# Harvard-AI-and-Robotics-Lab/FairFedMed

Measured on AMD Instinct MI355X. Metric: images/sec per client-round, ViT-B/16 FairLoRA r=8, bs=32 224^2, higher is better.
Workload: dtype bf16; 1 GPU; configs[1]: 1-client ViT-B/16 FairLoRA rank=8 G=3, bs=32 synthetic 224x224x3, fwd+bwd+SGD per step; global_batch=32, clients=1, trainable_elems=741952, loss_finite=1, launch=replay, rccl_ranks=1

## Files before the change

fairfedmed_amd/csrc/lora.hip:

```cpp
#include "common.h"

namespace {

constexpr int LD_WAVES = 8;
constexpr int LD_LDS_BUDGET = 64 * 1024;

template <int V>
__device__ __forceinline__ void reduce_scatter64(float (&vals)[V], int lane) {
#pragma unroll
    for (int n = V, o = 32; o >= 1; n >>= 1, o >>= 1) {
        const bool up = (lane & o) != 0;
#pragma unroll
        for (int i = 0; i < n / 2; ++i) {
            const float a = vals[i], b = vals[i + n / 2];
            const float keep = up ? b : a, send = up ? a : b;
            vals[i] = keep + __shfl_xor(send, o, 64);
        }
    }
}

template <typename T, int RP>
__global__ __launch_bounds__(LD_WAVES * 64) void lora_down_kernel(
    const T* __restrict__ x, int ldx, const float* __restrict__ P, int layout_rk, const float* __restrict__ S,
    const int32_t* __restrict__ attr, int M, int K, int r, int G, int rows_per_sample, float scaling,
// ... 226 lines not shown
        d_uni[e] = rows16(d_uni[e]);
    }
    if (col == 0) {
#pragma unroll
        for (int e = 0; e < 4; ++e) {
            dsum[0 * 16 + 4 * kgp + e] = d_all[e];
            dsum[1 * 16 + 4 * kgp + e] = d_uni[e];
        }
    }
    for (int g = 0; g < G; ++g) {
#pragma unroll
        for (int e = 0; e < 4; ++e) {
            const float o = rows16(ga == g ? wv[e] : 0.f);
            if (col == 0) dsum[(2 + g) * 16 + 4 * kgp + e] = o;
        }
    }
    __builtin_amdgcn_s_waitcnt(0xc07f);
    __builtin_amdgcn_wave_barrier();
    if (lane < G * r) {
        const int g = lane / r, j = lane % r;
        ds_part[((size_t)blockIdx.x * G + g) * r + j] = w_uni * dsum[16 + j] + w_oth * dsum[j] + (w_own - w_oth) * dsum[(2 + g) * 16 + j];
    }
    for (int i = lane + 64; i < G * r; i += 64) {
        const int g = i / r, j = i % r;
        ds_part[((size_t)blockIdx.x * G + g) * r + j] = w_uni * dsum[16 + j] + w_oth * dsum[j] + (w_own - w_oth) * dsum[(2 + g) * 16 + j];
    }
}

static bool down_mfma_ok(int M, int K, int r, int dtype, int layout_rk) {
    return dtype == FFM_BF16 && layout_rk && r <= 16 && M >= 1024 && K % (32 * LDM_WAVES) == 0;
}

static int down_kq(int K, int es) {
    const int nch = K * es / 16;
    return nch >= 256 ? 4 : nch >= 96 ? 2 : 1;
}
static int down_rp(int r, int dtype) { return r <= 4 && dtype == FFM_F32 ? 4 : r <= 8 ? 8 : 16; }

template <typename T, int RP>
int launch_down(const void* x, int ldx, const float* P, int layout_rk, const float* S, const int32_t* attr, int M,
                int K, int r, int G, int rps, float scaling, float lam, float* t, float* ts, const float* t_fwd,
                float* ds_part, int rs, int j0, hipStream_t s) {
    constexpr int CE = Elem<T>::kPerChunk;
    int ktile = K;
    const int per_col = RP * (int)sizeof(T);
    if (K * per_col > LD_LDS_BUDGET) ktile = (LD_LDS_BUDGET / per_col) / (64 * CE) * (64 * CE);
    const int lds = ktile * per_col;
    const int kq = down_kq(K, (int)sizeof(T));
    const int rows = (LD_WAVES / kq) * (64 / RP);
    const int blocks = (M + rows - 1) / rows;
    hipLaunchKernelGGL((lora_down_kernel<T, RP>), dim3(blocks), dim3(LD_WAVES * 64), lds, s, (const T*)x, ldx, P,
                       layout_rk, S, attr, M, K, r, G, rps, scaling, lam, t, ts, t_fwd, ds_part, ktile, rs, j0, kq);
    FFM_CHECK_LAUNCH();
    return FFM_OK;
}

constexpr int LG_WAVES = 4;
constexpr int LG_RPW = 32;
constexpr int LG_ROWS = LG_WAVES * LG_RPW;

template <typename T, int RP>
__global__ __launch_bounds__(LG_WAVES * 64) void lora_grad_kernel(const T* __restrict__ x, int ldx,
                                                                   const float* __restrict__ v, int M, int K, int r,
                                                                   float* __restrict__ part, int rs, int j0) {
    constexpr int CE = Elem<T>::kPerChunk;
    extern __shared__ __attribute__((aligned(16))) char smem[];
    float* red = reinterpret_cast<float*>(smem);
    const int lane = threadIdx.x & 63;
    const int wave = __builtin_amdgcn_readfirstlane(threadIdx.x >> 6);
    const int k = (blockIdx.x * 64 + lane) * CE;
    const int split = blockIdx.y;
    const bool active = k < K;
    const int m0 = split * LG_ROWS + wave * LG_RPW;
    const int m1 = (m0 + LG_RPW) < M ? (m0 + LG_RPW) : M;

    float acc[CE][RP];
#pragma unroll
    for (int e = 0; e < CE; ++e)
#pragma unroll
        for (int j = 0; j < RP; ++j) acc[e][j] = 0.f;

    const T* xc = x + (active ? k : 0);
    for (int m = m0; m < m1; m += 8) {
        typename Elem<T>::chunk_t xv[8];
#pragma unroll
        for (int u = 0; u < 8; ++u) {
            const int mm = (m + u) < m1 ? (m + u) : (m1 - 1);
            xv[u] = *reinterpret_cast<const typename Elem<T>::chunk_t*>(xc + (size_t)mm * ldx);
        }
#pragma unroll
        for (int u = 0; u < 8; ++u) {
            if (m + u < m1) {
                const float* vr = v + (size_t)(m + u) * rs + j0;
                float vj[RP];
#pragma unroll
                for (int j = 0; j < RP; ++j) vj[j] = (j < r) ? vr[j] : 0.f;
#pragma unroll
                for (int e = 0; e < CE; ++e) {
                    const float xe = Elem<T>::to_f(xv[u][e]);
#pragma unroll
                    for (int j = 0; j < RP; ++j) acc[e][j] += xe * vj[j];
                }
            }
        }
    }
    if (wave >= 2) {
#pragma unroll
        for (int e = 0; e < CE; ++e)
#pragma unroll
            for (int j = 0; j < RP; ++j) red[((wave - 2) * CE * RP + e * RP + j) * 64 + lane] = acc[e][j];
    }
    __syncthreads();
    if (wave < 2) {
#pragma unroll
        for (int e = 0; e < CE; ++e)
#pragma unroll
            for (int j = 0; j < RP; ++j) acc[e][j] += red[(wave * CE * RP + e * RP + j) * 64 + lane];
    }
    __syncthreads();
    if (wave == 1) {
#pragma unroll
        for (int e = 0; e < CE; ++e)
#pragma unroll
            for (int j = 0; j < RP; ++j) red[(e * RP + j) * 64 + lane] = acc[e][j];
    }
    __syncthreads();
    if (wave == 0 && active) {
        float* dst = part + ((size_t)split * K + k) * rs + j0;
#pragma unroll
        for (int e = 0; e < CE; ++e)
#pragma unroll
            for (int j = 0; j < RP; ++j)
                if (j < r) dst[e * rs + j] = acc[e][j] + red[(e * RP + j) * 64 + lane];
    }
}

template <typename T, int RP>
int launch_grad(const void* x, int ldx, const float* v, int M, int K, int r, float* part, int rs, int j0,
                hipStream_t s) {
    constexpr int CE = Elem<T>::kPerChunk;
    dim3 grid((K + 64 * CE - 1) / (64 * CE), (M + LG_ROWS - 1) / LG_ROWS);
    const int lds = 2 * CE * RP * 64 * 4;
    if (lds > 65536) {
        hipError_t e = hipFuncSetAttribute(reinterpret_cast<const void*>(lora_grad_kernel<T, RP>),
                                           hipFuncAttributeMaxDynamicSharedMemorySize, lds);
        if (e != hipSuccess) return (int)e;
    }
    hipLaunchKernelGGL((lora_grad_kernel<T, RP>), grid, dim3(LG_WAVES * 64), lds, s, (const T*)x, ldx, v, M, K, r,
                       part, rs, j0);
    FFM_CHECK_LAUNCH();
    return FFM_OK;
}

constexpr int LGM_ROWS = 128, LGM_COLS = 128;

__device__ __forceinline__ int lgm_swz(int row) { return ((row & 3) << 2) | ((row >> 2) & 3); }

struct lgm_ln {
    const float *mean, *rstd, *gamma, *beta;
};

template <int RP, bool LN>
__global__ __launch_bounds__(64) void lora_grad_mfma_kernel(const bf16_t* __restrict__ x, int ldx,
                                                            const float* __restrict__ v, int M, int K, int r,
                                                            float* __restrict__ part, int rs, int j0, lgm_ln ln) {
    extern __shared__ __attribute__((aligned(16))) char smem[];
    const int lane = threadIdx.x;
    const int k0 = blockIdx.x * LGM_COLS, split = blockIdx.y, m0 = split * LGM_ROWS;

#ifdef FFM_LGM_NOLDS
    {
        bf16x8 sink = {};
#pragma unroll 8
        for (int piece = 0; piece < LGM_ROWS / 4; ++piece) {
            const int row = piece * 4 + (lane >> 4);
            int gm = m0 + row;
            gm = gm < M ? gm : M - 1;
            const bf16x8 t = *reinterpret_cast<const bf16x8*>(x + (size_t)gm * ldx + k0 + (lane & 15) * 8);
#pragma unroll
            for (int e = 0; e < 8; ++e) sink[e] = (bf16_t)((float)sink[e] + (float)t[e]);
        }
        if (v[0] == 123456.f) part[lane] = (float)sink[0];
        return;
    }
#endif
#pragma unroll
    for (int piece = 0; piece < LGM_ROWS / 4; ++piece) {
        const int row = piece * 4 + (lane >> 4);
        int gm = m0 + row;
        gm = gm < M ? gm : M - 1;
        const int ch = (lane & 15) ^ lgm_swz(row);
        const bf16_t* src = x + (size_t)gm * ldx + k0 + ch * 8;
        __builtin_amdgcn_global_load_lds((const __attribute__((address_space(1))) void*)src,
                                         (__attribute__((address_space(3))) void*)(smem + piece * 1024), 16, 0, 0);
    }
    const int j = lane & 15, kg = lane >> 4;
    bf16x8 ahi[4], alo[4];
    float s1 = 0.f, s2 = 0.f;
#pragma unroll
    for (int rb = 0; rb < 4; ++rb) {
        float vv[8];
#pragma unroll
        for (int t = 0; t < 8; ++t) {
            const int gm = m0 + rb * 32 + kg * 8 + t;
            vv[t] = (j < r && gm < M) ? v[(size_t)gm * rs + j0 + j] : 0.f;
            if constexpr (LN) {
                const int gc = gm < M ? gm : M - 1;
                const float rsd = ln.rstd[gc];
                s2 += vv[t];
                vv[t] *= rsd;
                s1 += ln.mean[gc] * vv[t];
            }
        }
#pragma unroll
        for (int t = 0; t < 8; ++t) {
            const bf16_t h = (bf16_t)vv[t];
            ahi[rb][t] = h;
            alo[rb][t] = (bf16_t)(vv[t] - (float)h);
        }
    }
    asm volatile("s_waitcnt vmcnt(0)" ::: "memory");
    __builtin_amdgcn_s_barrier();

    const int q = (lane & 15) >> 2, pp = lane & 3;
    f32x4 acc[LGM_COLS / 16];
#pragma unroll
    for (int cf = 0; cf < LGM_COLS / 16; ++cf) acc[cf] = (f32x4){0.f, 0.f, 0.f, 0.f};
    typedef __attribute__((ext_vector_type(2))) uint32_t u32x2;
    typedef __attribute__((ext_vector_type(4))) uint32_t u32x4;
#pragma unroll
    for (int rb = 0; rb < 4; ++rb) {
        const int R = rb * 32 + kg * 8 + q;
        const uint32_t base0 = (uint32_t)(uintptr_t)smem + 256 * R + 8 * (pp & 1);
        const uint32_t base1 = base0 + 256 * 4;
        const int s0 = lgm_swz(R), s1 = lgm_swz(R + 4);
        u32x2 lo2[LGM_COLS / 16], hi2[LGM_COLS / 16];
#pragma unroll
        for (int cf = 0; cf < LGM_COLS / 16; ++cf) {
            const int ch = cf * 2 + (pp >> 1);
            asm volatile("ds_read_b64_tr_b16 %0, %1" : "=v"(lo2[cf]) : "v"(base0 + 16 * (ch ^ s0)) : "memory");
            asm volatile("ds_read_b64_tr_b16 %0, %1" : "=v"(hi2[cf]) : "v"(base1 + 16 * (ch ^ s1)) : "memory");
        }
        asm volatile("s_waitcnt lgkmcnt(0)" ::: "memory");
#pragma unroll
        for (int cf = 0; cf < LGM_COLS / 16; ++cf) {
            asm volatile("" : "+v"(lo2[cf]), "+v"(hi2[cf]));
            const u32x4 packed = {lo2[cf][0], lo2[cf][1], hi2[cf][0], hi2[cf][1]};
            const bf16x8 b = __builtin_bit_cast(bf16x8, packed);
            acc[cf] = __builtin_amdgcn_mfma_f32_16x16x32_bf16(ahi[rb], b, acc[cf], 0, 0, 0);
            acc[cf] = __builtin_amdgcn_mfma_f32_16x16x32_bf16(alo[rb], b, acc[cf], 0, 0, 0);
        }
    }
    (void)RP;
    float c1[4] = {0.f, 0.f, 0.f, 0.f}, c2[4] = {0.f, 0.f, 0.f, 0.f};
    if constexpr (LN) {
        s1 += __shfl_xor(s1, 16, 64);
        s1 += __shfl_xor(s1, 32, 64);
        s2 += __shfl_xor(s2, 16, 64);
        s2 += __shfl_xor(s2, 32, 64);
#pragma unroll
        for (int e = 0; e < 4; ++e) {
            c1[e] = __shfl(s1, 4 * kg + e, 64);
            c2[e] = __shfl(s2, 4 * kg + e, 64);
        }
    }
#pragma unroll
    for (int cf = 0; cf < LGM_COLS / 16; ++cf) {
        const int k = k0 + cf * 16 + (lane & 15);
        float* dst = part + ((size_t)split * K + k) * rs + j0;
        float gk = 1.f, bk = 0.f;
        if constexpr (LN) { gk = ln.gamma[k]; bk = ln.beta[k]; }
#pragma unroll
        for (int e = 0; e < 4; ++e) {
            const int jj = 4 * kg + e;
            if (jj < r) dst[jj] = LN ? gk * (acc[cf][e] - c1[e]) + bk * c2[e] : acc[cf][e];
        }
    }
}

int launch_grad_mfma(const void* x, int ldx, const float* v, int M, int K, int r, float* part, int rs, int j0,
                     hipStream_t s, const lgm_ln* ln = nullptr) {
    dim3 grid(K / LGM_COLS, (M + LGM_ROWS - 1) / LGM_ROWS);
#ifdef FFM_LGM_NOLDS
#define LGM_LDS 0
#else
#define LGM_LDS (LGM_ROWS * LGM_COLS * 2)
#endif
    if (ln)
        hipLaunchKernelGGL((lora_grad_mfma_kernel<16, true>), grid, dim3(64), LGM_LDS, s, (const bf16_t*)x, ldx,
                           v, M, K, r, part, rs, j0, *ln);
    else
        hipLaunchKernelGGL((lora_grad_mfma_kernel<16, false>), grid, dim3(64), LGM_LDS, s, (const bf16_t*)x, ldx,
                           v, M, K, r, part, rs, j0, lgm_ln{});
    FFM_CHECK_LAUNCH();
    return FFM_OK;
}

__global__ __launch_bounds__(256) void reduce_partials_kernel(const float* __restrict__ part, int nsplit, int n,
                                                              float* __restrict__ out, int tK, int tr,
                                                              int accumulate) {
    const int gid = blockIdx.x * blockDim.x + threadIdx.x;
    const int i = (gid >> 2);
    const int q = gid & 3;
    float s = 0.f;
    if (i < n)
        for (int sp = q; sp < nsplit; sp += 4) s += part[(size_t)sp * n + i];
    s += __shfl_xor(s, 1, 64);
    s += __shfl_xor(s, 2, 64);
    if (i >= n || q != 0) return;
    int o = i;
    if (tK > 0) {
        const int k = i / tr, j = i % tr;
        o = j * tK + k;
    }
    out[o] = accumulate ? out[o] + s : s;
}

__global__ __launch_bounds__(1024) void reduce_partials_tall_kernel(const float* __restrict__ part, int nsplit, int n,
                                                                    float* __restrict__ out, int tK, int tr, int accumulate) {
    __shared__ float red[16][64];
    const int lane = threadIdx.x & 63, wave = threadIdx.x >> 6;
    const int i = blockIdx.x * 64 + lane;
    float s0 = 0.f, s1 = 0.f, s2 = 0.f, s3 = 0.f;
    if (i < n) {
        int sp = wave;
        for (; sp + 48 < nsplit; sp += 64) {
            s0 += part[(size_t)sp * n + i];
            s1 += part[(size_t)(sp + 16) * n + i];
            s2 += part[(size_t)(sp + 32) * n + i];
            s3 += part[(size_t)(sp + 48) * n + i];
        }
        for (; sp < nsplit; sp += 16) s0 += part[(size_t)sp * n + i];
    }
    red[wave][lane] = (s0 + s1) + (s2 + s3);
    __syncthreads();
    if (wave != 0 || i >= n) return;
    float s = 0.f;
#pragma unroll
    for (int w = 0; w < 16; ++w) s += red[w][lane];
    int o = i;
    if (tK > 0) {
        const int k = i / tr, j = i % tr;
        o = j * tK + k;
    }
    out[o] = accumulate ? out[o] + s : s;
}

__global__ __launch_bounds__(256) void reduce_multi_kernel(const ffm_reduce_desc* __restrict__ descs) {
    const ffm_reduce_desc d = descs[blockIdx.y];
    const int L = d.nsplit > 64 ? 32 : 4, sh = d.nsplit > 64 ? 5 : 2;
    if ((long long)blockIdx.x * blockDim.x >= (long long)L * d.n) return;
    const int gid = blockIdx.x * blockDim.x + threadIdx.x;
    const int i = gid >> sh, q = gid & (L - 1);
    float s = 0.f;
    if (i < d.n)
        for (int sp = q; sp < d.nsplit; sp += L) s += d.part[(size_t)sp * d.n + i];
    s += __shfl_xor(s, 1, 64);
    s += __shfl_xor(s, 2, 64);
    if (L == 32) {
        s += __shfl_xor(s, 4, 64);
        s += __shfl_xor(s, 8, 64);
        s += __shfl_xor(s, 16, 64);
    }
    if (i >= d.n || q != 0) return;
    int o = i;
    if (d.transpose_K > 0) {
        const int k = i / d.transpose_r, j = i % d.transpose_r;
        o = j * d.transpose_K + k;
    }
    d.out[o] = s;
}

}

static int down_valu_blocks(int M, int K, int r, int dtype) {
    const int rows = (LD_WAVES / down_kq(K, dtype == FFM_BF16 ? 2 : 4)) * (64 / down_rp(r, dtype));
    return (M + rows - 1) / rows;
}
extern "C" int ffm_lora_down_blocks(int M, int K, int r, int dtype) {
    if (down_mfma_ok(M, K, r, dtype, 1)) return (M + LDM_ROWS - 1) / LDM_ROWS;
    return down_valu_blocks(M, K, r, dtype);
}
extern "C" int ffm_lora_down_blocks_max(int M_max, int K, int r, int dtype) {
    const int valu = down_valu_blocks(M_max, K, r, dtype);
    const int mf = down_mfma_ok(M_max, K, r, dtype, 1) ? (M_max + LDM_ROWS - 1) / LDM_ROWS : 0;
    return mf > valu ? mf : valu;
}
extern "C" int ffm_lora_grad_splits(int M) { return (M + LG_ROWS - 1) / LG_ROWS; }

extern "C" int ffm_lora_down(const void* x, int ldx, const float* P, int layout_rk, const float* S,
                             const int32_t* attr, int M, int K, int r, int G, int rows_per_sample, float scaling,
                             float lambda_group, float* t, float* ts, const float* t_fwd, float* ds_part, int dtype,
                             void* stream) {
    if (!x || !P || !S || M <= 0 || K <= 0 || r <= 0 || r > FFM_MAX_RANK || G <= 0 || G > FFM_MAX_GROUPS ||
        rows_per_sample <= 0)
        return FFM_EINVAL;
    if ((t_fwd == nullptr) != (ds_part == nullptr)) return FFM_EINVAL;
    if (G * r > 256) return FFM_EUNSUP;
    const size_t es = dtype == FFM_BF16 ? 2 : 4;
    if (dtype != FFM_BF16 && dtype != FFM_F32) return FFM_EINVAL;
    if (((size_t)K * es) % 16 || ((size_t)ldx * es) % 16 || ((uintptr_t)x & 15)) return FFM_EINVAL;
    hipStream_t s = (hipStream_t)stream;
    if (down_mfma_ok(M, K, r, dtype, layout_rk)) {
        hipLaunchKernelGGL(lora_down_mfma_kernel, dim3((M + LDM_ROWS - 1) / LDM_ROWS), dim3(LDM_WAVES * 64), 0, s, (const bf16_t*)x,
                           ldx, P, S, attr, M, K, r, G, rows_per_sample, scaling, lambda_group, t, ts, t_fwd, ds_part);
        FFM_CHECK_LAUNCH();
        return FFM_OK;
    }
#define DOWN(RP, RR, J0) launch_down<T, RP>(x, ldx, P, layout_rk, S, attr, M, K, RR, G, rows_per_sample, scaling, \
                                            lambda_group, t, ts, t_fwd, ds_part, r, J0, s)
    return ffm_by_storage(dtype, [&](auto tag) {
        typedef typename decltype(tag)::type T;
        if (r > 16) {
            int e = DOWN(16, 16, 0);
            if (e) return e;
            return DOWN(16, r - 16, 16);
        }
        if constexpr (sizeof(T) == 4) {
            if (r <= 4) return DOWN(4, r, 0);
        }
        return r <= 8 ? DOWN(8, r, 0) : DOWN(16, r, 0);
    });
#undef DOWN
}

extern "C" int ffm_lora_grad_partial(const void* x, int ldx, const float* v, int M, int K, int r, float* part,
                                     int dtype, void* stream) {
    if (!x || !v || !part || M <= 0 || K <= 0 || r <= 0 || r > FFM_MAX_RANK) return FFM_EINVAL;
    const size_t es = dtype == FFM_BF16 ? 2 : 4;
    if (dtype != FFM_BF16 && dtype != FFM_F32) return FFM_EINVAL;
    if (((size_t)K * es) % 16 || ((size_t)ldx * es) % 16 || ((uintptr_t)x & 15)) return FFM_EINVAL;
    hipStream_t s = (hipStream_t)stream;
    if (dtype == FFM_BF16 && K % LGM_COLS == 0) {
        for (int j0 = 0; j0 < r; j0 += 16) {
            const int e = launch_grad_mfma(x, ldx, v, M, K, (r - j0) < 16 ? (r - j0) : 16, part, r, j0, s);
            if (e) return e;
        }
        return FFM_OK;
    }
#define GRAD(RP, RR, J0) launch_grad<T, RP>(x, ldx, v, M, K, RR, part, r, J0, s)
    return ffm_by_storage(dtype, [&](auto tag) {
        typedef typename decltype(tag)::type T;
        if (r > 16) {
            int e = GRAD(16, 16, 0);
            if (e) return e;
            return GRAD(16, r - 16, 16);
        }
        return r <= 4 ? GRAD(4, r, 0) : r <= 8 ? GRAD(8, r, 0) : GRAD(16, r, 0);
    });
#undef GRAD
}

extern "C" int ffm_lora_grad_partial_ln(const void* x, int ldx, const float* v, const float* mean, const float* rstd,
                                        const float* gamma, const float* beta, int M, int K, int r, float* part,
                                        int dtype, void* stream) {
    if (!x || !v || !mean || !rstd || !gamma || !beta || !part || M <= 0 || K <= 0 || r <= 0) return FFM_EINVAL;
    if (dtype != FFM_BF16 || K % LGM_COLS || r > 16) return FFM_EUNSUP;
    if (((size_t)ldx * 2) % 16 || ((uintptr_t)x & 15)) return FFM_EINVAL;
    const lgm_ln ln = {mean, rstd, gamma, beta};
    return launch_grad_mfma(x, ldx, v, M, K, r, part, r, 0, (hipStream_t)stream, &ln);
}

extern "C" int ffm_reduce_partials_multi(const ffm_reduce_desc* descs_dev, int ndesc, int max_n, void* stream) {
    if (!descs_dev || ndesc <= 0 || max_n <= 0) return FFM_EINVAL;
    hipLaunchKernelGGL(reduce_multi_kernel, dim3((4 * max_n + 255) / 256, ndesc), dim3(256), 0, (hipStream_t)stream,
                       descs_dev);
    FFM_CHECK_LAUNCH();
    return FFM_OK;
}

extern "C" int ffm_reduce_partials(const float* part, int nsplit, int n, float* out, int transpose_K,
                                   int transpose_r, int accumulate, void* stream) {
    if (!part || !out || nsplit <= 0 || n <= 0) return FFM_EINVAL;
    if (transpose_K > 0 && (transpose_r <= 0 || transpose_K * transpose_r != n)) return FFM_EINVAL;
    if (nsplit >= 512 && (long long)n * 16 < (long long)nsplit * 64)
        hipLaunchKernelGGL(reduce_partials_tall_kernel, dim3((n + 63) / 64), dim3(1024), 0, (hipStream_t)stream, part, nsplit, n,
                           out, transpose_K, transpose_r, accumulate);
    else
        hipLaunchKernelGGL(reduce_partials_kernel, dim3((4 * n + 255) / 256), dim3(256), 0, (hipStream_t)stream, part,
                           nsplit, n, out, transpose_K, transpose_r, accumulate);
    FFM_CHECK_LAUNCH();
    return FFM_OK;
}
```

fairfedmed_amd/ops.py:

```python
from __future__ import annotations

import ctypes as C
from typing import Optional

import torch

from . import _lib as L

Tensor = torch.Tensor

_REC = None


class record:
    def __init__(self, plan: list):
        self.plan = plan

    def __enter__(self):
        global _REC
        self.prev, _REC = _REC, self.plan
        return self.plan

    def __exit__(self, *a):
        global _REC
# ... 513 lines not shown
    _call("ffm_eval_counts", L.ptr(prob), L.ptr(label), L.ptr(attr), N, num_groups, L.ptr(out), L.stream_ptr())
    return out


EVAL_BOOT_WS_BUDGET = 256 << 20
EVAL_BOOT_MAX_CHUNK = 65535


def eval_boot_chunk(N: int, B: int) -> int:
    size = L.load().ffm_eval_boot_ws_bytes
    if int(size(N, 1)) <= 0:
        raise RuntimeError("ffm_eval_boot_ws_bytes failed")
    lo, hi = 1, int(max(1, min(B, EVAL_BOOT_MAX_CHUNK)))
    while lo < hi:
        mid = (lo + hi + 1) // 2
        if int(size(N, mid)) <= EVAL_BOOT_WS_BUDGET:
            lo = mid
        else:
            hi = mid - 1
    return lo


def eval_boot_counts(prob: Tensor, label: Tensor, attr: Optional[Tensor], num_groups: int, B: int, seed: int, tag: int = 0,
                     chunk: Optional[int] = None, out: Optional[Tensor] = None) -> Tensor:
    _dev(prob, label, attr)
    N = prob.shape[0]
    assert prob.dtype == torch.float32 and prob.dim() == 2 and prob.shape[1] == 2 and prob.is_contiguous()
    assert label.dtype == torch.int64 and label.is_contiguous() and label.numel() == N
    assert attr is None or (attr.dtype == torch.int64 and attr.is_contiguous() and attr.numel() == N)
    B = int(B)
    if B <= 0:
        raise ValueError(f"eval_boot_counts needs B >= 1 replicates, got {B}")
    if recording():
        raise RuntimeError("eval_boot_counts holds a temporary workspace and cannot be recorded")
    if chunk is None:
        chunk = eval_boot_chunk(N, B)
    chunk = int(chunk)
    if not 1 <= chunk <= EVAL_BOOT_MAX_CHUNK:
        raise ValueError(f"eval_boot_counts: chunk must lie in 1..{EVAL_BOOT_MAX_CHUNK}, got {chunk}")
    if out is None:
        out = torch.empty(B, num_groups + 2, EVAL_SLOTS, device=prob.device, dtype=torch.int64)
    assert out.dtype == torch.int64 and out.is_contiguous() and tuple(out.shape) == (B, num_groups + 2, EVAL_SLOTS) and out.is_cuda
    nbytes = int(L.load().ffm_eval_boot_ws_bytes(N, chunk))
    if nbytes <= 0:
        raise RuntimeError("ffm_eval_boot_ws_bytes failed")
    ws = torch.empty(nbytes + 256, device=prob.device, dtype=torch.uint8)
    off = (-ws.data_ptr()) % 256
    _call("ffm_eval_boot_counts", L.ptr(prob), L.ptr(label), L.ptr(attr), N, num_groups, B, chunk, int(seed), int(tag),
          L.ptr(out), ws.data_ptr() + off, nbytes, L.stream_ptr())
    return out


def attention_fwd(qkv: Tensor, out: Tensor, lse: Optional[Tensor], B: int, Ltok: int, heads: int,
                  causal: bool = False) -> Tensor:
    _dev(qkv, out, lse)
    assert qkv.is_contiguous() and out.is_contiguous() and qkv.dtype == out.dtype
    assert qkv.shape[1] == 3 * heads * 64 and out.shape[1] == heads * 64
    _call("ffm_attention_fwd", L.ptr(qkv), L.ptr(out), L.ptr(_f32(lse)), B, Ltok, heads, int(causal),
                                       L.dtype_code(qkv.dtype), L.stream_ptr())
    return out


def attention_bwd_lnstat_ok(Ltok: int, causal: bool, dtype: torch.dtype) -> bool:
    return L.is16(dtype) and bool(L.load().ffm_attention_bwd_lnstat_ok(Ltok, int(causal), L.dtype_code(dtype)))


def attention_bwd(qkv: Tensor, out: Tensor, dout: Tensor, lse: Tensor, delta: Tensor, dqkv: Tensor, B: int,
                  Ltok: int, heads: int, causal: bool = False, ln_stat: Optional[tuple] = None) -> Tensor:
    _dev(qkv, out, dout, lse, delta, dqkv)
    for t in (qkv, out, dout, dqkv):
        assert t.is_contiguous() and t.dtype == qkv.dtype
    if ln_stat is not None:
        wg, d, part = ln_stat
        _dev(wg, d, part)
        E3 = 3 * heads * 64
        assert _f32(wg).numel() == E3 and _f32(d).numel() == E3 and _f32(part).numel() >= 2 * heads * B * Ltok * 2
        _call("ffm_attention_bwd_lnstat", L.ptr(qkv), L.ptr(out), L.ptr(dout), L.ptr(_f32(lse)), L.ptr(_f32(delta)), L.ptr(dqkv),
              L.ptr(wg), L.ptr(d), L.ptr(part), B, Ltok, heads, int(causal), L.dtype_code(qkv.dtype), L.stream_ptr())
        return dqkv
    _call("ffm_attention_bwd", L.ptr(qkv), L.ptr(out), L.ptr(dout), L.ptr(_f32(lse)), L.ptr(_f32(delta)),
                                       L.ptr(dqkv), B, Ltok, heads, int(causal), L.dtype_code(qkv.dtype),
                                       L.stream_ptr())
    return dqkv


def lora_down_blocks(M: int, K: int, r: int, dtype: torch.dtype) -> int:
    return L.load().ffm_lora_down_blocks(M, K, r, L.dtype_code(dtype))


def lora_down_blocks_max(M_max: int, K: int, r: int, dtype: torch.dtype) -> int:
    return L.load().ffm_lora_down_blocks_max(M_max, K, r, L.dtype_code(dtype))


class ReducePlan:

    def __init__(self, entries, device):
        import ctypes as C
        arr = (L.ReduceDesc * len(entries))()
        self.keep = entries
        self.max_n = 0
        for i, (part, nsplit, n, out, tK, tr) in enumerate(entries):
            _dev(part, out)
            arr[i] = L.ReduceDesc(part.data_ptr(), out.data_ptr(), nsplit, n, tK, tr)
            self.max_n = max(self.max_n, n * (8 if nsplit > 64 else 1))
        raw = bytes(arr)
        self.table = torch.frombuffer(bytearray(raw), dtype=torch.uint8).to(device)
        self.n = len(entries)

    def run(self) -> None:
        _call("ffm_reduce_partials_multi", self.table.data_ptr(), self.n, self.max_n, L.stream_ptr())


class PackPlan:

    def __init__(self, entries, dtype, device):
        arr = (L.PackDesc * len(entries))()
        self.keep, self.max_K, self.dtype = entries, 0, dtype
        self.any_ln = False
        for i, ent in enumerate(entries):
            src, layout_rk, dst = ent[:3]
            wide = ent[3] if len(ent) > 3 else None
            ln = ent[4] if len(ent) > 4 else None
            _dev(src, dst, wide)
            K = dst.shape[1]
            r = src.shape[0] if layout_rk else src.shape[1]
            assert dst.dtype == dtype and dst.shape[0] == 16 and dst.is_contiguous() and src.is_contiguous()
            assert wide is None or (wide.dtype == dtype and tuple(wide.shape) == (K, 32) and wide.is_contiguous())
            lnp = (None, None, None)
            if ln is not None:
                assert not layout_rk and _f32(ln[0]).numel() == K and _f32(ln[1]).numel() == K and _f32(ln[2]).numel() == 32
                _dev(*ln)
                lnp = tuple(t.data_ptr() for t in ln)
                self.any_ln = True
            rows = ent[5] if len(ent) > 5 and ent[5] is not None else (None, None)
            if rows[0] is not None:
                _dev(*rows)
                assert r <= 14 and _f32(rows[0]).numel() == K and _f32(rows[1]).numel() == K
            arr[i] = L.PackDesc(src.data_ptr(), dst.data_ptr(), K, r, int(layout_rk), 0, L.ptr(wide), *lnp, L.ptr(rows[0]), L.ptr(rows[1]))
            self.max_K = max(self.max_K, K)
        self.table = torch.frombuffer(bytearray(bytes(arr)), dtype=torch.uint8).to(device)
        self.n = len(entries)

    def run(self) -> None:
        _call("ffm_lora_pack_multi", self.table.data_ptr(), self.n, self.max_K, L.dtype_code(self.dtype),
                                             L.stream_ptr())
        if self.any_ln:
            _call("ffm_lora_pack_ln", self.table.data_ptr(), self.n, L.dtype_code(self.dtype), L.stream_ptr())


def lora_grad_partial_ln(x: Tensor, v: Tensor, mean: Tensor, rstd: Tensor, gamma: Tensor, beta: Tensor, r: int,
                         part: Tensor) -> None:
    _dev(x, v, mean, rstd, gamma, beta, part)
    M, K = x.shape
    assert L.is16(x.dtype) and K % 128 == 0 and r <= 16
    _call("ffm_lora_grad_partial_ln", L.ptr(x), _ld(x), L.ptr(_f32(v)), L.ptr(_f32(mean)), L.ptr(_f32(rstd)),
          L.ptr(_f32(gamma)), L.ptr(_f32(beta)), M, K, r, L.ptr(_f32(part)), L.dtype_code(x.dtype), L.stream_ptr())


def lora_grad_splits(M: int) -> int:
    return L.load().ffm_lora_grad_splits(M)


def lora_down(x: Tensor, P: Tensor, layout_rk: bool, S: Tensor, attr: Optional[Tensor], r: int, G: int,
              rows_per_sample: int, scaling: float, lambda_group: float, t: Optional[Tensor], ts: Optional[Tensor],
              t_fwd: Optional[Tensor] = None, ds_part: Optional[Tensor] = None) -> None:
    _dev(x, P, S, attr, t, ts, t_fwd, ds_part)
    M, K = x.shape
    if attr is not None:
        assert attr.dtype == torch.int32
    _call("ffm_lora_down", L.ptr(x), _ld(x), L.ptr(_f32(P)), int(layout_rk), L.ptr(_f32(S)), L.ptr(attr), M,
                                   K, r, G, rows_per_sample, scaling, lambda_group, L.ptr(_f32(t)), L.ptr(_f32(ts)),
                                   L.ptr(_f32(t_fwd)), L.ptr(_f32(ds_part)), L.dtype_code(x.dtype), L.stream_ptr())


def lora_grad_partial(x: Tensor, v: Tensor, r: int, part: Tensor) -> None:
    _dev(x, v, part)
    M, K = x.shape
    _call("ffm_lora_grad_partial", L.ptr(x), _ld(x), L.ptr(_f32(v)), M, K, r, L.ptr(_f32(part)),
                                           L.dtype_code(x.dtype), L.stream_ptr())


def reduce_partials(part: Tensor, nsplit: int, n: int, out: Tensor, transpose_K: int = 0, transpose_r: int = 0,
                    accumulate: bool = False) -> None:
    _dev(part, out)
    _call("ffm_reduce_partials", L.ptr(_f32(part)), nsplit, n, L.ptr(out), transpose_K, transpose_r,
                                         int(accumulate), L.stream_ptr())


def head_fwd(f: Tensor, tbar: Tensor, logit_scale: Tensor, fbar: Tensor, rnorm: Tensor, logits_img: Tensor, B: int,
             Ltok: int, n_cls: int) -> None:
    _dev(f, tbar, logit_scale, fbar, rnorm, logits_img)
    D = f.shape[1]
    assert f.is_contiguous()
    _call("ffm_head_fwd", L.ptr(f), L.ptr(_f32(tbar)), L.ptr(_f32(logit_scale)), L.ptr(_f32(fbar)),
                                  L.ptr(_f32(rnorm)), L.ptr(_f32(logits_img)), B, Ltok, D, n_cls,
                                  L.dtype_code(f.dtype), L.stream_ptr())


def text_embed(prefix: Tensor, ctx: Tensor, suffix: Tensor, pos: Tensor, x: Tensor, n_cls: int, TL: int) -> None:
    _dev(prefix, ctx, suffix, pos, x)
    n_prompts, n_ctx, w = ctx.shape
    for t in (prefix, ctx, suffix, pos, x):
        assert t.dtype == torch.float32 and t.is_contiguous()
    assert prefix.shape[0] == suffix.shape[0] == n_prompts * n_cls and x.shape[0] >= n_prompts * n_cls * TL and pos.shape[0] >= TL
    _call("ffm_text_embed", L.ptr(prefix), L.ptr(ctx), L.ptr(suffix), suffix.shape[1], L.ptr(pos), L.ptr(x), n_prompts, n_cls,
          n_ctx, TL, w, L.stream_ptr())


def text_tail_fwd(x: Tensor, eot_row: Tensor, lnw: Tensor, lnb: Tensor, proj: Tensor, tf: Tensor, tn: Tensor, rnorm: Tensor,
                  stats: Tensor, tbar: Optional[Tensor], n_prompts: int, n_cls: int) -> None:
    _dev(x, eot_row, lnw, lnb, proj, tf, tn, rnorm, stats, tbar)
    assert eot_row.dtype == torch.int32 and x.dtype == torch.float32 and proj.dtype == torch.float32 and proj.is_contiguous()
    w, D = proj.shape
    assert x.shape[1] == w and tf.shape == tn.shape == (n_prompts * n_cls, D) and tf.is_contiguous() and tn.is_contiguous()
    _call("ffm_text_tail_fwd", L.ptr(x), L.ptr(eot_row), L.ptr(lnw), L.ptr(lnb), L.ptr(proj), L.ptr(tf), L.ptr(tn), L.ptr(rnorm),
          L.ptr(stats), L.ptr(tbar), n_prompts, n_cls, w, D, L.stream_ptr())


def text_tail_bwd(x: Tensor, eot_row: Tensor, lnw: Tensor, proj: Tensor, tn: Tensor, rnorm: Tensor, stats: Tensor,
                  dtbar: Optional[Tensor], dtn: Optional[Tensor], dy: Tensor, g: Tensor, n_prompts: int, n_cls: int, TL: int) -> None:
    _dev(x, eot_row, lnw, proj, tn, rnorm, stats, dtbar, dtn, dy, g)
    w, D = proj.shape
    assert g.dtype == torch.float32 and g.is_contiguous() and g.shape[0] >= n_prompts * n_cls * TL and g.shape[1] == w
    _call("ffm_text_tail_bwd", L.ptr(x), L.ptr(eot_row), L.ptr(lnw), L.ptr(proj), L.ptr(tn), L.ptr(rnorm), L.ptr(stats),
          L.ptr(dtbar), L.ptr(dtn), L.ptr(dy), L.ptr(g), n_prompts, n_cls, TL, w, D, L.stream_ptr())


def text_ctx_grad(g: Tensor, dctx: Tensor, n_cls: int, TL: int) -> None:
    _dev(g, dctx)
    n_prompts, n_ctx, w = dctx.shape
    assert g.dtype == dctx.dtype == torch.float32 and g.is_contiguous() and dctx.is_contiguous()
    _call("ffm_text_ctx_grad", L.ptr(g), L.ptr(dctx), n_prompts, n_cls, n_ctx, TL, w, L.stream_ptr())


def ce_loss(logits_img: Tensor, label: Tensor, logits: Tensor, prob: Tensor, loss: Tensor, dlogits_img: Tensor,
            finite: Optional[Tensor], nb: int, S: int, n_cls: int) -> None:
    _dev(logits_img, label, logits, prob, loss, dlogits_img, finite)
    assert label.dtype == torch.int64 and (finite is None or finite.dtype == torch.int32)
    _call("ffm_ce_loss", L.ptr(_f32(logits_img)), L.ptr(label), L.ptr(_f32(logits)), L.ptr(_f32(prob)),
                                 L.ptr(_f32(loss)), L.ptr(_f32(dlogits_img)), L.ptr(finite), nb, S, n_cls,
                                 L.stream_ptr())


def ce_fair_loss(logits_img: Tensor, label: Tensor, attr: Tensor, logits: Tensor, prob: Tensor, loss: Tensor,
                 terms: Tensor, gstat: Optional[Tensor], dlogits_img: Tensor, finite: Optional[Tensor], nb: int, S: int,
                 n_cls: int, G: int, lam: float, with_grad: bool = False) -> None:
    _dev(logits_img, label, attr, logits, prob, loss, terms, gstat, dlogits_img, finite)
    assert label.dtype == torch.int64 and attr.dtype == torch.int32 and (finite is None or finite.dtype == torch.int32)
    assert attr.is_contiguous() and attr.numel() >= nb and label.numel() >= nb and terms.numel() >= 2
    assert logits_img.numel() >= nb * S * n_cls and dlogits_img.numel() >= nb * S * n_cls
    assert logits.numel() >= nb * n_cls and prob.numel() >= nb * n_cls and (gstat is None or gstat.numel() >= 2 * G)
    _call("ffm_ce_fair_loss", L.ptr(_f32(logits_img)), L.ptr(label), L.ptr(attr), L.ptr(_f32(logits)), L.ptr(_f32(prob)),
          L.ptr(_f32(loss)), L.ptr(_f32(terms)), L.ptr(_f32(gstat)), L.ptr(_f32(dlogits_img)), L.ptr(finite), nb, S,
          n_cls, G, float(lam), int(bool(with_grad)), L.stream_ptr())


def head_bwd(f: Tensor, tbar: Tensor, logit_scale: Tensor, fbar: Tensor, rnorm: Tensor, dlogits_img: Tensor,
             df: Tensor, dtbar: Tensor, B: int, Ltok: int, n_cls: int) -> None:
    _dev(f, tbar, logit_scale, fbar, rnorm, dlogits_img, df, dtbar)
    D = f.shape[1]
    assert f.dtype == df.dtype and df.is_contiguous()
    _call("ffm_head_bwd", L.ptr(f), L.ptr(_f32(tbar)), L.ptr(_f32(logit_scale)), L.ptr(_f32(fbar)),
                                  L.ptr(_f32(rnorm)), L.ptr(_f32(dlogits_img)), L.ptr(df), L.ptr(_f32(dtbar)), B,
                                  Ltok, D, n_cls, L.dtype_code(f.dtype), L.stream_ptr())


def sgd_momentum(p: Tensor, g: Tensor, buf: Tensor, lr: float, momentum: float, weight_decay: float,
                 first_step: bool, repeats: int = 1) -> None:
    _dev(p, g, buf)
    if repeats == 1:
        _call("ffm_sgd_momentum", L.ptr(_f32(p)), L.ptr(_f32(g)), L.ptr(_f32(buf)), p.numel(), lr, momentum,
              weight_decay, int(first_step), L.stream_ptr())
    else:
        _call("ffm_sgd_momentum_n", L.ptr(_f32(p)), L.ptr(_f32(g)), L.ptr(_f32(buf)), p.numel(), lr, momentum,
              weight_decay, int(first_step), int(repeats), L.stream_ptr())


MAX_GROUPS = 8
SCALE_STATE = 8


def loss_scale(p: Tensor, state: Tensor) -> None:
    _dev(p, state)
    assert p.is_contiguous() and state.numel() == SCALE_STATE
    _call("ffm_loss_scale", L.ptr(_f32(p)), p.numel(), L.ptr(_f32(state)), L.stream_ptr())


def unscale_check(g: Tensor, state: Tensor) -> None:
    _dev(g, state)
    assert g.is_contiguous() and state.numel() == SCALE_STATE
    _call("ffm_unscale_check", L.ptr(_f32(g)), g.numel(), L.ptr(_f32(state)), L.stream_ptr())


def sgd_momentum_gated(p: Tensor, g: Tensor, buf: Tensor, lr: float, momentum: float, weight_decay: float,
                       first_step: bool, repeats: int, state: Tensor) -> None:
    _dev(p, g, buf, state)
    _call("ffm_sgd_momentum_gated", L.ptr(_f32(p)), L.ptr(_f32(g)), L.ptr(_f32(buf)), p.numel(), lr, momentum,
          weight_decay, int(first_step), int(repeats), L.ptr(_f32(state)), L.stream_ptr())


def sgd_momentum_dev(p: Tensor, g: Tensor, buf: Tensor, hp: Tensor, repeats: int = 1,
                     state: Optional[Tensor] = None) -> None:
    _dev(p, g, buf, hp, state)
    assert state is None or state.numel() == SCALE_STATE
    _call("ffm_sgd_momentum_dev", L.ptr(_f32(p)), L.ptr(_f32(g)), L.ptr(_f32(buf)), p.numel(), L.ptr(_f32(hp)),
          int(repeats), L.ptr(_f32(state)), L.stream_ptr())

# ... 126 lines not shown
```

Measured before the change: 7070 images/sec.

## Pipeline LoRA grad MFMA kernel over multiple 64-column tiles per block

Restructures the LoRA weight-gradient MFMA kernel so each single-wave block handles up to two 64-column tiles. The activation loads and LDS transposes are split into quarters, and the next tile's global-to-LDS loads are issued while the current tile's MFMAs run. The v, mean and rstd operands are loaded once per block and reused across tiles, with LayerNorm stats fetched per lane and broadcast by shuffles. The LDS tile shrinks and uses a new swizzle, and debug-only paths are removed. This adds 32-bit pitch offsets, which require a new ldx limit check, and puts more barrier and waitcnt logic on a hot backward kernel.

```diff
diff --git a/fairfedmed_amd/csrc/lora.hip b/fairfedmed_amd/csrc/lora.hip
--- a/fairfedmed_amd/csrc/lora.hip
+++ b/fairfedmed_amd/csrc/lora.hip
@@ -402,9 +402,67 @@
     return FFM_OK;
 }
 
-constexpr int LGM_ROWS = 128, LGM_COLS = 128;
-
-__device__ __forceinline__ int lgm_swz(int row) { return ((row & 3) << 2) | ((row >> 2) & 3); }
+constexpr int LGM_ROWS = 128, LGM_COLS = 64, LGM_TPB = 2;
+constexpr int LGM_LDS = LGM_ROWS * LGM_COLS * 2, LGM_QUARTER = LGM_LDS / 4;
+constexpr int LGM_MAX_LDX = 1 << 23;
+
+__device__ __forceinline__ int lgm_swz(int row) { return (((row >> 1) & 1) << 1) | (((row >> 3) & 1) << 2); }
+
+__device__ __forceinline__ void lgm_issue(const char* tile, uint32_t pitch, int rows, int qd, char* smem, int lane) {
+    if (rows >= LGM_ROWS) {
+#pragma unroll
+        for (int pi = 0; pi < 4; ++pi) {
+            const uint32_t off = (uint32_t)(lane >> 3) * pitch + 16u * (uint32_t)((lane & 7) ^ lgm_swz(pi * 8 + (lane >> 3)));
+            const char* piece = tile + (size_t)(qd * 32 + pi * 8) * pitch;
+            __builtin_amdgcn_global_load_lds((const __attribute__((address_space(1))) void*)(piece + off),
+                                             (__attribute__((address_space(3))) void*)(smem + qd * LGM_QUARTER + pi * 1024), 16, 0, 0);
+        }
+        return;
+    }
+#pragma unroll
+    for (int pi = 0; pi < 4; ++pi) {
+        const int row = qd * 32 + pi * 8 + (lane >> 3);
+        const int rl = row < rows ? row : rows - 1;
+        const uint32_t off = (uint32_t)rl * pitch + 16u * (uint32_t)((lane & 7) ^ lgm_swz(row));
+        __builtin_amdgcn_global_load_lds((const __attribute__((address_space(1))) void*)(tile + off),
+                                         (__attribute__((address_space(3))) void*)(smem + qd * LGM_QUARTER + pi * 1024), 16, 0, 0);
+    }
+}
+
+typedef __attribute__((ext_vector_type(2))) uint32_t lgm_u32x2;
+template <int N> __device__ __forceinline__ void lgm_wait_vm() { asm volatile("s_waitcnt vmcnt(%0)" ::"n"(N) : "memory"); }
+template <int OFF> __device__ __forceinline__ lgm_u32x2 lgm_tr_read(uint32_t a) {
+    lgm_u32x2 d;
+    asm volatile("ds_read_b64_tr_b16 %0, %1 offset:%2" : "=v"(d) : "v"(a), "n"(OFF) : "memory");
+    return d;
+}
+
+template <int QD>
+__device__ __forceinline__ void lgm_quarter(bool wait, bool next, const uint32_t (&la)[LGM_COLS / 16], const bf16x8& ah,
+                                            const bf16x8& al, f32x4 (&acc)[LGM_COLS / 16], const char* tile_next,
+                                            uint32_t pitch, int rows, char* smem, int lane) {
+    typedef __attribute__((ext_vector_type(4))) uint32_t u32x4;
+    if (wait) {
+        if (next) lgm_wait_vm<12>(); else lgm_wait_vm<4 * (3 - QD)>();
+        __builtin_amdgcn_s_barrier();
+    }
+    lgm_u32x2 lo2[LGM_COLS / 16], hi2[LGM_COLS / 16];
+#pragma unroll
+    for (int cf = 0; cf < LGM_COLS / 16; ++cf) {
+        lo2[cf] = lgm_tr_read<QD * LGM_QUARTER>(la[cf]);
+        hi2[cf] = lgm_tr_read<QD * LGM_QUARTER + 4 * 2 * LGM_COLS>(la[cf]);
+    }
+    asm volatile("s_waitcnt lgkmcnt(0)" ::: "memory");
+    if (next) lgm_issue(tile_next, pitch, rows, QD, smem, lane);
+#pragma unroll
+    for (int cf = 0; cf < LGM_COLS / 16; ++cf) {
+        asm volatile("" : "+v"(lo2[cf]), "+v"(hi2[cf]));
+        const u32x4 packed = {lo2[cf][0], lo2[cf][1], hi2[cf][0], hi2[cf][1]};
+        const bf16x8 b = __builtin_bit_cast(bf16x8, packed);
+        acc[cf] = __builtin_amdgcn_mfma_f32_16x16x32_bf16(ah, b, acc[cf], 0, 0, 0);
+        acc[cf] = __builtin_amdgcn_mfma_f32_16x16x32_bf16(al, b, acc[cf], 0, 0, 0);
+    }
+}
 
 struct lgm_ln {
     const float *mean, *rstd, *gamma, *beta;
@@ -413,92 +471,60 @@
 template <int RP, bool LN>
 __global__ __launch_bounds__(64) void lora_grad_mfma_kernel(const bf16_t* __restrict__ x, int ldx,
                                                             const float* __restrict__ v, int M, int K, int r,
-                                                            float* __restrict__ part, int rs, int j0, lgm_ln ln) {
+                                                            float* __restrict__ part, int rs, int j0, lgm_ln ln,
+                                                            int tpb) {
     extern __shared__ __attribute__((aligned(16))) char smem[];
     const int lane = threadIdx.x;
-    const int k0 = blockIdx.x * LGM_COLS, split = blockIdx.y, m0 = split * LGM_ROWS;
-
-#ifdef FFM_LGM_NOLDS
-    {
-        bf16x8 sink = {};
-#pragma unroll 8
-        for (int piece = 0; piece < LGM_ROWS / 4; ++piece) {
-            const int row = piece * 4 + (lane >> 4);
-            int gm = m0 + row;
-            gm = gm < M ? gm : M - 1;
-            const bf16x8 t = *reinterpret_cast<const bf16x8*>(x + (size_t)gm * ldx + k0 + (lane & 15) * 8);
-#pragma unroll
-            for (int e = 0; e < 8; ++e) sink[e] = (bf16_t)((float)sink[e] + (float)t[e]);
-        }
-        if (v[0] == 123456.f) part[lane] = (float)sink[0];
-        return;
-    }
-#endif
-#pragma unroll
-    for (int piece = 0; piece < LGM_ROWS / 4; ++piece) {
-        const int row = piece * 4 + (lane >> 4);
-        int gm = m0 + row;
-        gm = gm < M ? gm : M - 1;
-        const int ch = (lane & 15) ^ lgm_swz(row);
-        const bf16_t* src = x + (size_t)gm * ldx + k0 + ch * 8;
-        __builtin_amdgcn_global_load_lds((const __attribute__((address_space(1))) void*)src,
-                                         (__attribute__((address_space(3))) void*)(smem + piece * 1024), 16, 0, 0);
+    const int split = blockIdx.y, m0 = split * LGM_ROWS;
+    const int k0 = blockIdx.x * tpb * LGM_COLS;
+    const int left = K / LGM_COLS - blockIdx.x * tpb, nt = left < tpb ? left : tpb;
+
+    const uint32_t pitch = (uint32_t)ldx * 2u;
+    const int rows = M - m0;
+    const char* tile0 = reinterpret_cast<const char*>(x + (size_t)m0 * ldx + k0);
+#pragma unroll
+    for (int qd = 0; qd < 4; ++qd) lgm_issue(tile0, pitch, rows, qd, smem, lane);
+    float rs2[2] = {0.f, 0.f}, mu2[2] = {0.f, 0.f}, gl[LGM_TPB], bl[LGM_TPB];
+    if constexpr (LN) {
+#pragma unroll
+        for (int h = 0; h < 2; ++h) {
+            const int gm = m0 + 64 * h + lane, gc = gm < M ? gm : M - 1;
+            rs2[h] = ln.rstd[gc];
+            mu2[h] = ln.mean[gc];
+        }
+#pragma unroll
+        for (int g = 0; g < LGM_TPB; ++g) {
+            const int k = k0 + (g < nt ? g : 0) * LGM_COLS + lane;
+            gl[g] = ln.gamma[k];
+            bl[g] = ln.beta[k];
+        }
     }
     const int j = lane & 15, kg = lane >> 4;
     bf16x8 ahi[4], alo[4];
     float s1 = 0.f, s2 = 0.f;
+    const float* vb = v + (size_t)m0 * rs + j0;
+    const uint32_t vl = (uint32_t)(kg * 8) * (uint32_t)rs + (uint32_t)j;
 #pragma unroll
     for (int rb = 0; rb < 4; ++rb) {
         float vv[8];
 #pragma unroll
         for (int t = 0; t < 8; ++t) {
             const int gm = m0 + rb * 32 + kg * 8 + t;
-            vv[t] = (j < r && gm < M) ? v[(size_t)gm * rs + j0 + j] : 0.f;
+            const float* vrow = vb + (size_t)(rb * 32 + t) * rs;
+            vv[t] = (j < r && gm < M) ? vrow[vl] : 0.f;
+        }
+#pragma unroll
+        for (int t = 0; t < 8; ++t) {
             if constexpr (LN) {
-                const int gc = gm < M ? gm : M - 1;
-                const float rsd = ln.rstd[gc];
+                const int src = (rb & 1) * 32 + kg * 8 + t;
+                const float rsd = __shfl(rs2[rb >> 1], src, 64);
                 s2 += vv[t];
                 vv[t] *= rsd;
-                s1 += ln.mean[gc] * vv[t];
-            }
-        }
-#pragma unroll
-        for (int t = 0; t < 8; ++t) {
+                s1 = __builtin_fmaf(__shfl(mu2[rb >> 1], src, 64), vv[t], s1);
+            }
             const bf16_t h = (bf16_t)vv[t];
             ahi[rb][t] = h;
             alo[rb][t] = (bf16_t)(vv[t] - (float)h);
-        }
-    }
-    asm volatile("s_waitcnt vmcnt(0)" ::: "memory");
-    __builtin_amdgcn_s_barrier();
-
-    const int q = (lane & 15) >> 2, pp = lane & 3;
-    f32x4 acc[LGM_COLS / 16];
-#pragma unroll
-    for (int cf = 0; cf < LGM_COLS / 16; ++cf) acc[cf] = (f32x4){0.f, 0.f, 0.f, 0.f};
-    typedef __attribute__((ext_vector_type(2))) uint32_t u32x2;
-    typedef __attribute__((ext_vector_type(4))) uint32_t u32x4;
-#pragma unroll
-    for (int rb = 0; rb < 4; ++rb) {
-        const int R = rb * 32 + kg * 8 + q;
-        const uint32_t base0 = (uint32_t)(uintptr_t)smem + 256 * R + 8 * (pp & 1);
-        const uint32_t base1 = base0 + 256 * 4;
-        const int s0 = lgm_swz(R), s1 = lgm_swz(R + 4);
-        u32x2 lo2[LGM_COLS / 16], hi2[LGM_COLS / 16];
-#pragma unroll
-        for (int cf = 0; cf < LGM_COLS / 16; ++cf) {
-            const int ch = cf * 2 + (pp >> 1);
-            asm volatile("ds_read_b64_tr_b16 %0, %1" : "=v"(lo2[cf]) : "v"(base0 + 16 * (ch ^ s0)) : "memory");
-            asm volatile("ds_read_b64_tr_b16 %0, %1" : "=v"(hi2[cf]) : "v"(base1 + 16 * (ch ^ s1)) : "memory");
-        }
-        asm volatile("s_waitcnt lgkmcnt(0)" ::: "memory");
-#pragma unroll
-        for (int cf = 0; cf < LGM_COLS / 16; ++cf) {
-            asm volatile("" : "+v"(lo2[cf]), "+v"(hi2[cf]));
-            const u32x4 packed = {lo2[cf][0], lo2[cf][1], hi2[cf][0], hi2[cf][1]};
-            const bf16x8 b = __builtin_bit_cast(bf16x8, packed);
-            acc[cf] = __builtin_amdgcn_mfma_f32_16x16x32_bf16(ahi[rb], b, acc[cf], 0, 0, 0);
-            acc[cf] = __builtin_amdgcn_mfma_f32_16x16x32_bf16(alo[rb], b, acc[cf], 0, 0, 0);
         }
     }
     (void)RP;
@@ -513,38 +539,74 @@
             c1[e] = __shfl(s1, 4 * kg + e, 64);
             c2[e] = __shfl(s2, 4 * kg + e, 64);
         }
-    }
-#pragma unroll
-    for (int cf = 0; cf < LGM_COLS / 16; ++cf) {
-        const int k = k0 + cf * 16 + (lane & 15);
-        float* dst = part + ((size_t)split * K + k) * rs + j0;
-        float gk = 1.f, bk = 0.f;
-        if constexpr (LN) { gk = ln.gamma[k]; bk = ln.beta[k]; }
-#pragma unroll
-        for (int e = 0; e < 4; ++e) {
-            const int jj = 4 * kg + e;
-            if (jj < r) dst[jj] = LN ? gk * (acc[cf][e] - c1[e]) + bk * c2[e] : acc[cf][e];
-        }
-    }
+#pragma unroll
+        for (int g = 0; g < LGM_TPB; ++g) asm volatile("" : "+v"(gl[g]), "+v"(bl[g]));
+    }
+    asm volatile("s_waitcnt vmcnt(0)" ::: "memory");
+    __builtin_amdgcn_s_barrier();
+
+    const int q = (lane & 15) >> 2, pp = lane & 3;
+    const int sp = ((q >> 1) & 1) | ((kg & 1) << 1);
+    uint32_t la[LGM_COLS / 16];
+#pragma unroll
+    for (int cf = 0; cf < LGM_COLS / 16; ++cf)
+        la[cf] = (uint32_t)(uintptr_t)smem + 2 * LGM_COLS * (kg * 8 + q) + 32 * (cf ^ sp) + 8 * pp;
+#pragma unroll 1
+    for (int g = 0; g < nt; ++g) {
+        const bool next = g + 1 < nt;
+        const char* tn = tile0 + (g + 1) * (LGM_COLS * 2);
+        f32x4 acc[LGM_COLS / 16];
+#pragma unroll
+        for (int cf = 0; cf < LGM_COLS / 16; ++cf) acc[cf] = (f32x4){0.f, 0.f, 0.f, 0.f};
+        lgm_quarter<0>(g > 0, next, la, ahi[0], alo[0], acc, tn, pitch, rows, smem, lane);
+        lgm_quarter<1>(g > 0, next, la, ahi[1], alo[1], acc, tn, pitch, rows, smem, lane);
+        lgm_quarter<2>(g > 0, next, la, ahi[2], alo[2], acc, tn, pitch, rows, smem, lane);
+        lgm_quarter<3>(g > 0, next, la, ahi[3], alo[3], acc, tn, pitch, rows, smem, lane);
+        float glg = 1.f, blg = 0.f;
+        if constexpr (LN) {
+#pragma unroll
+            for (int i = 0; i < LGM_TPB; ++i) {
+                glg = g == i ? gl[i] : glg;
+                blg = g == i ? bl[i] : blg;
+            }
+        }
+#pragma unroll
+        for (int cf = 0; cf < LGM_COLS / 16; ++cf) {
+            const int k = k0 + g * LGM_COLS + cf * 16 + (lane & 15);
+            float* dst = part + ((size_t)split * K + k) * rs + j0;
+            float gk = 1.f, bk = 0.f;
+            if constexpr (LN) {
+                gk = __shfl(glg, cf * 16 + (lane & 15), 64);
+                bk = __shfl(blg, cf * 16 + (lane & 15), 64);
+            }
+#pragma unroll
+            for (int e = 0; e < 4; ++e) {
+                const int jj = 4 * kg + e;
+                if (jj < r) dst[jj] = LN ? __builtin_fmaf(bk, c2[e], gk * (acc[cf][e] - c1[e])) : acc[cf][e];
+            }
+        }
+    }
+}
+
+inline int lgm_tpb(int K) {
+    const int tiles = K / LGM_COLS, blocks = (tiles + LGM_TPB - 1) / LGM_TPB;
+    return (tiles + blocks - 1) / blocks;
 }
 
 int launch_grad_mfma(const void* x, int ldx, const float* v, int M, int K, int r, float* part, int rs, int j0,
                      hipStream_t s, const lgm_ln* ln = nullptr) {
-    dim3 grid(K / LGM_COLS, (M + LGM_ROWS - 1) / LGM_ROWS);
-#ifdef FFM_LGM_NOLDS
-#define LGM_LDS 0
-#else
-#define LGM_LDS (LGM_ROWS * LGM_COLS * 2)
-#endif
+    const int tpb = lgm_tpb(K);
+    dim3 grid((K / LGM_COLS + tpb - 1) / tpb, (M + LGM_ROWS - 1) / LGM_ROWS);
     if (ln)
         hipLaunchKernelGGL((lora_grad_mfma_kernel<16, true>), grid, dim3(64), LGM_LDS, s, (const bf16_t*)x, ldx,
-                           v, M, K, r, part, rs, j0, *ln);
+                           v, M, K, r, part, rs, j0, *ln, tpb);
     else
         hipLaunchKernelGGL((lora_grad_mfma_kernel<16, false>), grid, dim3(64), LGM_LDS, s, (const bf16_t*)x, ldx,
-                           v, M, K, r, part, rs, j0, lgm_ln{});
+                           v, M, K, r, part, rs, j0, lgm_ln{}, tpb);
     FFM_CHECK_LAUNCH();
     return FFM_OK;
 }
+
 
 __global__ __launch_bounds__(256) void reduce_partials_kernel(const float* __restrict__ part, int nsplit, int n,
                                                               float* __restrict__ out, int tK, int tr,
@@ -681,7 +743,7 @@
     if (dtype != FFM_BF16 && dtype != FFM_F32) return FFM_EINVAL;
     if (((size_t)K * es) % 16 || ((size_t)ldx * es) % 16 || ((uintptr_t)x & 15)) return FFM_EINVAL;
     hipStream_t s = (hipStream_t)stream;
-    if (dtype == FFM_BF16 && K % LGM_COLS == 0) {
+    if (dtype == FFM_BF16 && K % LGM_COLS == 0 && ldx < LGM_MAX_LDX) {
         for (int j0 = 0; j0 < r; j0 += 16) {
             const int e = launch_grad_mfma(x, ldx, v, M, K, (r - j0) < 16 ? (r - j0) : 16, part, r, j0, s);
             if (e) return e;
@@ -705,7 +767,7 @@
                                         const float* gamma, const float* beta, int M, int K, int r, float* part,
                                         int dtype, void* stream) {
     if (!x || !v || !mean || !rstd || !gamma || !beta || !part || M <= 0 || K <= 0 || r <= 0) return FFM_EINVAL;
-    if (dtype != FFM_BF16 || K % LGM_COLS || r > 16) return FFM_EUNSUP;
+    if (dtype != FFM_BF16 || K % LGM_COLS || r > 16 || ldx >= LGM_MAX_LDX) return FFM_EUNSUP;
     if (((size_t)ldx * 2) % 16 || ((uintptr_t)x & 15)) return FFM_EINVAL;
     const lgm_ln ln = {mean, rstd, gamma, beta};
     return launch_grad_mfma(x, ldx, v, M, K, r, part, r, 0, (hipStream_t)stream, &ln);
diff --git a/fairfedmed_amd/ops.py b/fairfedmed_amd/ops.py
--- a/fairfedmed_amd/ops.py
+++ b/fairfedmed_amd/ops.py
@@ -689,7 +689,7 @@
                          part: Tensor) -> None:
     _dev(x, v, mean, rstd, gamma, beta, part)
     M, K = x.shape
-    assert L.is16(x.dtype) and K % 128 == 0 and r <= 16
+    assert L.is16(x.dtype) and K % 64 == 0 and r <= 16
     _call("ffm_lora_grad_partial_ln", L.ptr(x), _ld(x), L.ptr(_f32(v)), L.ptr(_f32(mean)), L.ptr(_f32(rstd)),
           L.ptr(_f32(gamma)), L.ptr(_f32(beta)), M, K, r, L.ptr(_f32(part)), L.dtype_code(x.dtype), L.stream_ptr())
 
```

After: 7087 images/sec, median of 2. Within noise of the previous version (+0.3%).
